# MiniXC/LightningFastSpeech2

Hardware: AMD Instinct MI355X
Metric: mel-frames/sec (whole node), 256-phoneme batch-32 (higher is better)
Workload: dtype bf16

## Files before the change

### include/fs2.h

```cpp
#ifndef FS2_H_
#define FS2_H_

#include <stddef.h>
#include <stdint.h>

#ifdef __cplusplus
extern "C" {
#endif

#define FS2_ABI_VERSION 4
#define FS2_MAX_LAYERS 32
#define FS2_MAX_VARIANCES 4
#define FS2_MAX_PRIORS 8
#define FS2_NAME_LEN 32

enum fs2_status {
    FS2_OK = 0,
    FS2_ERR_HIP = 1,
    FS2_ERR_SHAPE = 2,
    FS2_ERR_ARG = 3,
    FS2_ERR_WEIGHT = 4,
    FS2_ERR_STATE = 5,
    FS2_ERR_NOMEM = 6
};
// ... 105 lines not shown
int32_t fs2_op_vocoder_resblock_form(int32_t dtype, int32_t channels, int32_t taps, const int32_t* dilations, int32_t npairs);
int32_t fs2_op_vocoder_conv_tile(int32_t dtype, int32_t n, int32_t cin, int32_t taps, int32_t dil, int32_t shift, int32_t post,
                                 int32_t* cin_pad);
int fs2_op_gemm(int32_t dtype, int32_t out_dtype, const void* x, const void* w, const float* bias, void* c,
                int32_t M, int32_t N, int32_t Cin, int32_t taps, int32_t S, int32_t relu, void* hip_stream);
int fs2_op_gemm_relu_dropout(int32_t dtype, const void* x, const void* w, const float* bias, void* c, int32_t M, int32_t N, int32_t Cin,
                             int32_t taps, int32_t S, float p, uint64_t seed, uint64_t key, void* hip_stream);
int fs2_op_gemm_add(int32_t dtype, const void* x, const void* w, const float* bias, const void* addend, void* c, int32_t M, int32_t N,
                    int32_t Cin, int32_t taps, int32_t S, void* hip_stream);
int fs2_op_gemm_rowscale(const void* x, const void* w, const float* bias, const float* rowstats, const float* wg,
                         void* c, int32_t M, int32_t N, int32_t Cin, void* hip_stream);
int fs2_op_gemm_rowscale_dt(int32_t dtype, int32_t out_dtype, const void* x, const void* w, const float* bias, const float* rowstats,
                            const float* wg, void* c, int32_t M, int32_t N, int32_t Cin, void* hip_stream);
int fs2_op_gemm_stats(int32_t dtype, const void* x, const void* w, const float* bias, const void* res, void* c, float* stats, int32_t M,
                      int32_t N, int32_t Cin, int32_t relu, void* hip_stream);
int fs2_op_rowstats_finish(const float* parts, int32_t nparts, int32_t ncols, float eps, float* out, int32_t M, void* hip_stream);
int fs2_op_gemm_head(const void* x, const void* w, const float* bias, const float* head_gw, float* stats_out, float* head_out, int32_t M,
                     int32_t N, int32_t Cin, int32_t relu, void* hip_stream);
int fs2_op_head_finish(const float* parts, const float* dots, int32_t nparts, int32_t ncols, float eps, float sum_gw, float cst,
                       const uint8_t* mask, float* pred, int32_t M, void* hip_stream);
int fs2_op_gemm_splitk_choice(int32_t dtype, int32_t M, int32_t N, int32_t Cin, int32_t taps, int32_t S);
int32_t fs2_op_gemm_route(int32_t dtype, int32_t out_dtype, int32_t M, int32_t N, int32_t Cin, int32_t taps, int32_t S, int32_t ksplit,
                          uint32_t present, int32_t bias_aligned);
int fs2_op_gemm_splitk(int32_t dtype, int32_t out_dtype, const void* x, const void* w, void* c, float* part, int32_t M, int32_t N,
                       int32_t Cin, int32_t taps, int32_t S, int32_t ksplit, int32_t accumulate, void* hip_stream);
int fs2_op_gemm_gated(int32_t dtype, const void* x, const void* w, const float* bias, const void* gate, float scale, void* c,
                      int32_t M, int32_t N, int32_t Cin, int32_t taps, int32_t S, void* hip_stream);
int fs2_op_attention(int32_t dtype, const void* qkv, const uint8_t* key_pad_mask, void* out, void* vt_scratch,
                     uint64_t* bits_scratch, int32_t B, int32_t S, int32_t H, int32_t heads, void* hip_stream);
int fs2_op_attention_x3(const float* qkv, const uint8_t* key_pad_mask, float* out, void* split_scratch, uint64_t* bits_scratch,
                        int32_t B, int32_t S, int32_t H, int32_t heads, void* hip_stream);
int fs2_op_gemm_split_out(const void* x, const void* w, const float* bias, void* c_hi, void* c_lo, int32_t M, int32_t N, int32_t Cin,
                          int32_t split, void* hip_stream);
int fs2_op_gemm_ln(int32_t dtype, const void* x, const void* w, const float* bias, const void* res,
                   const float* ln_g, const float* ln_b, const float* dot_w, float dot_b, const uint8_t* mask,
                   float* pred, void* y, void* tmp, int32_t M, int32_t N, int32_t Cin, int32_t taps, int32_t S,
                   int32_t relu, void* hip_stream);
int fs2_op_gemm_ln_tape(int32_t dtype, const void* x, const void* w, const float* bias, const void* res, const float* ln_g,
                        const float* ln_b, void* y, void* z_out, int32_t M, int32_t N, int32_t Cin, int32_t taps, int32_t S,
                        int32_t relu, void* hip_stream);
int fs2_op_gemm_ln_tape_dropout(int32_t dtype, const void* x, const void* w, const float* bias, const void* res, const float* ln_g,
                                const float* ln_b, void* y, void* z_out, int32_t M, int32_t N, int32_t Cin, int32_t taps, int32_t S,
                                int32_t relu, float p, uint64_t seed, uint64_t key, void* hip_stream);
size_t fs2_op_attention_scratch_bytes(int32_t dtype, int32_t B, int32_t S, int32_t H, int32_t heads, size_t* bits_bytes);
int fs2_op_layernorm(int32_t dtype, const void* x, const void* res, const float* gamma, const float* beta, void* y,
                     const float* dot_w, float dot_b, const uint8_t* mask, float* pred, int32_t M, int32_t H,
// ... 243 lines not shown
```

### lightningfastspeech2_amd/csrc/capi_ops.hip

```cpp
#include <math.h>

#include "fs2_common.h"
#include "fs2_kernels.h"

using namespace fs2;

namespace fs2 {

template <typename S, typename D>
__global__ __launch_bounds__(256) void convert_kernel(const S* __restrict__ s, D* __restrict__ d, size_t n) {
    for (size_t i = (size_t)blockIdx.x * 256 + threadIdx.x; i < n; i += (size_t)gridDim.x * 256)
        d[i] = Num<D>::from_f32(Num<S>::to_f32(s[i]));
}

int launch_convert(const ConvertArgs& a, int sdt, int ddt, hipStream_t st) {
    if (a.n == 0) return FS2_OK;
    size_t blocks = (a.n + 255) / 256;
    if (blocks > 4096) blocks = 4096;
    const dim3 g((unsigned)blocks), b(256);
    if (sdt == FS2_F32 && ddt == FS2_F32) hipLaunchKernelGGL((convert_kernel<float, float>), g, b, 0, st, (const float*)a.src, (float*)a.dst, a.n);
    else if (sdt == FS2_F32 && ddt == FS2_BF16) hipLaunchKernelGGL((convert_kernel<float, bf16>), g, b, 0, st, (const float*)a.src, (bf16*)a.dst, a.n);
    else if (sdt == FS2_BF16 && ddt == FS2_F32) hipLaunchKernelGGL((convert_kernel<bf16, float>), g, b, 0, st, (const bf16*)a.src, (float*)a.dst, a.n);
    else if (sdt == FS2_BF16 && ddt == FS2_BF16) hipLaunchKernelGGL((convert_kernel<bf16, bf16>), g, b, 0, st, (const bf16*)a.src, (bf16*)a.dst, a.n);
    else if (sdt == FS2_F32 && ddt == FS2_F16) hipLaunchKernelGGL((convert_kernel<float, f16>), g, b, 0, st, (const float*)a.src, (f16*)a.dst, a.n);
// ... 4 lines not shown
}

}

namespace fs2 {
int apply_knob(Tuning& t, int variant) {
    int ok = 1;
    if (variant == 1500 || variant == 1501) t.attn_x3 = variant - 1500;
    else if (variant >= 1400 && variant <= 1402) t.gemm_wres = variant - 1400;
    else if (variant == 1340 || variant == 1341) t.enc_attn_out = variant - 1340;
    else if (variant == 1320 || variant == 1321) t.pred_fuse_embed = variant - 1320;
    else if (variant >= 1200 && variant <= 1204) t.attn_pipe = variant - 1200;
    else if (variant == 1100 || variant == 1101) t.colsum_fused = variant - 1100;
    else if (variant == 1000 || variant == 1001) t.bgemm_tn256 = variant - 1000;
    else if (variant >= 905 && variant <= 908) { if (variant >= 907) t.attn_bwd_nb_dq = 3 + ((variant - 905) & 1); else t.attn_bwd_nb = 3 + ((variant - 905) & 1); }
    else if (variant == 909) t.attn_bwd_nb = 1;
    else if (variant >= 900 && variant <= 903) { if (variant >= 902) t.attn_bwd_nb_dq = ((variant - 900) & 1) + 1; else t.attn_bwd_nb = ((variant - 900) & 1) + 1; }
    else if (variant == 904) t.attn_bwd_nb_dq = 0;
    else if (variant == 800 || variant == 801) t.bgemm_full = variant - 800;
    else if (variant == 700 || variant == 701) t.bgemm_xcd = variant - 700;
    else if (variant == 500 || variant == 501) t.split_f32 = variant - 500;
    else if (variant == 230 || variant == 231) t.head_sums = variant - 230;
    else if (variant == 220 || variant == 221) t.gemm_persist = variant - 220;
    else if (variant >= 200 && variant <= 202) t.slab_xcd_remap = variant - 200;
    else if (variant >= 0 && variant <= 7 && variant != 2) t.gemm_variant = variant;
    else ok = 0;
    if (!ok) return FS2_ERR_ARG;
    ++t.gen;
    return FS2_OK;
}
Tuning& op_tuning() {
    static thread_local Tuning t;
    return t;
}
}

static GemmArgs gemm_args(const void* x, const void* w, const float* bias, void* c, int M, int N, int Cin, int taps, int S, int relu) {
    GemmArgs a;
    a.X = x; a.W = w; a.bias = bias; a.C = c;
    a.M = M; a.N = N; a.K = taps * Cin; a.ldx = Cin; a.ldc = N;
    a.Cin = Cin; a.taps = taps; a.pad = (taps - 1) / 2; a.S = S; a.relu = relu;
    return a;
}

extern "C" {

// ... 122 lines not shown
    GemmArgs a = gemm_args(x, w, bias, c, M, N, Cin, 1, M, 0);
    a.rs_stats = rowstats; a.rs_wg = wg;
    return launch_gemm(a, dtype, out_dtype, (hipStream_t)stream);
}
int fs2_op_rowstats_finish(const float* parts, int32_t nparts, int32_t ncols, float eps, float* out, int32_t M, void* stream) {
    return launch_rowstats_finish(parts, nparts, ncols, eps, out, M, (hipStream_t)stream);
}
int fs2_op_gemm_head(const void* x, const void* w, const float* bias, const float* head_gw, float* stats_out, float* head_out, int32_t M,
                     int32_t N, int32_t Cin, int32_t relu, void* stream) {
    if (!x || !w || !bias || !head_gw || !stats_out || !head_out) return FS2_ERR_ARG;
    GemmArgs a = gemm_args(x, w, bias, nullptr, M, N, Cin, 1, M, relu);
    a.stats_out = stats_out; a.head_gw = head_gw; a.head_out = head_out; a.ln_eps = 1e-5f;
    return launch_gemm(a, FS2_BF16, FS2_BF16, (hipStream_t)stream);
}
int fs2_op_head_finish(const float* parts, const float* dots, int32_t nparts, int32_t ncols, float eps, float sum_gw, float cst,
                       const uint8_t* mask, float* pred, int32_t M, void* stream) {
    return launch_head_finish(parts, dots, nparts, ncols, eps, sum_gw, cst, mask, pred, M, (hipStream_t)stream);
}

int fs2_op_gemm_splitk_choice(int32_t dtype, int32_t M, int32_t N, int32_t Cin, int32_t taps, int32_t S) {
    return gemm_splitk_choice(M, N, Cin, taps, S, dtype);
}

int32_t fs2_op_gemm_route(int32_t dtype, int32_t out_dtype, int32_t M, int32_t N, int32_t Cin, int32_t taps, int32_t S, int32_t ksplit,
                          uint32_t present, int32_t bias_aligned) {
    static float dummy[8];
    void* p = (void*)(((uintptr_t)dummy + 15) & ~(uintptr_t)15);
    GemmArgs a = gemm_args(p, p, nullptr, p, M, N, Cin, taps, S, (present & GF_RELU) != 0);
    a.ksplit = ksplit;
    if (present & GF_BIAS) a.bias = (const float*)p + (bias_aligned ? 0 : 1);
    if (present & GF_RES) a.res = p;
    if (present & GF_LN) { a.ln_g = (const float*)p; a.ln_b = (const float*)p; }
    if (present & GF_DOT) a.dot_w = (const float*)p;
    if (present & GF_ZOUT) a.z_out = p;
    if (present & GF_LNTMP) a.ln_tmp = p;
    if (present & GF_STATS) a.stats_out = (float*)p;
    if (present & GF_EPIRES) a.epi_res = p;
    if (present & GF_GATE) a.gate = p;
    if (present & GF_DROP) a.drop_p = 0.1f;
    if (present & GF_RS) { a.rs_stats = (const float*)p; a.rs_wg = (const float*)p; }
    if (present & GF_HEAD) { a.head_out = (float*)p; a.head_gw = (const float*)p; }
    if (present & GF_ZR) a.zero_rows = (const uint8_t*)p;
    if (present & GF_CLO) a.C_lo = p;
    if (present & GF_SPLIT) a.split = 1;
    if (present & GF_WPRE) a.w_presplit = 1;
    const GemmRoute r = route_gemm(a, dtype, out_dtype);
    if (r.status != FS2_OK) return -r.status;
    return r.family | r.mi << 4 | (r.ln ? 1 : 0) << 8 | (r.split ? 1 : 0) << 9 | (r.defer ? 1 : 0) << 10 | (r.xpre ? 1 : 0) << 11 |
           (r.zr ? 1 : 0) << 12 | (r.presplit ? 1 : 0) << 13 | (r.two_launch ? 1 : 0) << 16;
}

int fs2_op_gemm_splitk(int32_t dtype, int32_t out_dtype, const void* x, const void* w, void* c, float* part, int32_t M, int32_t N,
                       int32_t Cin, int32_t taps, int32_t S, int32_t ksplit, int32_t accumulate, void* stream) {
    if (ksplit < 2 || !part) return FS2_ERR_ARG;
    GemmArgs a = gemm_args(x, w, nullptr, part, M, N, Cin, taps, S, 0);
    a.ksplit = ksplit;
    const int r = launch_gemm(a, dtype, FS2_F32, (hipStream_t)stream);
    if (r != FS2_OK) return r;
    return launch_split_k_reduce(part, c, (size_t)M * N, ksplit, accumulate, out_dtype, (hipStream_t)stream);
}

int fs2_op_gemm_gated(int32_t dtype, const void* x, const void* w, const float* bias, const void* gate, float scale, void* c, int32_t M,
                      int32_t N, int32_t Cin, int32_t taps, int32_t S, void* stream) {
    if (!gate) return FS2_ERR_ARG;
    GemmArgs a = gemm_args(x, w, bias, c, M, N, Cin, taps, S, 0);
    a.gate = gate; a.gate_scale = scale;
    return launch_gemm(a, dtype, dtype, (hipStream_t)stream);
}

int fs2_op_gemm_ln(int32_t dtype, const void* x, const void* w, const float* bias, const void* res,
                   const float* ln_g, const float* ln_b, const float* dot_w, float dot_b, const uint8_t* mask,
                   float* pred, void* y, void* tmp, int32_t M, int32_t N, int32_t Cin, int32_t taps, int32_t S,
// ... 399 lines not shown
```

### lightningfastspeech2_amd/csrc/fs2_kernels.h

```cpp
#pragma once
#include <hip/hip_runtime.h>
#include <stdint.h>

#include <type_traits>

#include "../../include/fs2.h"
#include "fs2_common.h"

namespace fs2 {

inline bool is_16bit(int dt) { return dt == FS2_BF16 || dt == FS2_F16; }
inline bool is_storage_dtype(int dt) { return dt == FS2_F32 || is_16bit(dt); }
inline bool is_f32_or_bf16(int dt) { return dt == FS2_F32 || dt == FS2_BF16; }
inline size_t elem_bytes(int dt) { return is_16bit(dt) ? 2 : 4; }

struct Tuning {
    int gemm_variant = 0;
    int gemm_wres = 1;
    int head_sums = 1;
    int gemm_persist = 1;
    int slab_xcd_remap = 1;
    int split_f32 = 0;
    int attn_pipe = 3;
    int attn_x3 = 1;
    int enc_attn_out = 1;
    int pred_fuse_embed = 1;
    int attn_bwd_nb = 1, attn_bwd_nb_dq = 0;
    int colsum_fused = 0;
    int bgemm_full = 1, bgemm_xcd = 1, bgemm_tn256 = 1;
    int voc_lds_limit = 0;
    int voc_fused_resblock = 1;
    unsigned long long gen = 0;
};
Tuning& op_tuning();
int apply_knob(Tuning& t, int variant);
inline const Tuning& tuning_of(const Tuning* t) { return t ? *t : op_tuning(); }

struct GemmArgs {
    const void* X;
    const void* W;
    const float* bias;
    void* C;
    void* C_lo = nullptr;
    int M, N, K;
// ... 22 lines not shown
    int w_presplit = 0;
    int split = 0;
    const uint8_t* zero_rows = nullptr;
    const void* gate = nullptr;
    float gate_scale = 1.f;
    float drop_p = 0.f;
    uint64_t drop_seed = 0, drop_key = 0;
    const float* rs_stats = nullptr;
    const float* rs_wg = nullptr;
    const float* head_gw = nullptr;
    float* head_out = nullptr;
    int ksplit = 0;
};
enum GemmFeature : unsigned {
    GF_BIAS = 1u << 0, GF_RES = 1u << 1, GF_LN = 1u << 2, GF_DOT = 1u << 3, GF_ZOUT = 1u << 4, GF_LNTMP = 1u << 5, GF_STATS = 1u << 6,
    GF_EPIRES = 1u << 7, GF_GATE = 1u << 8, GF_DROP = 1u << 9, GF_RS = 1u << 10 , GF_HEAD = 1u << 11 ,
    GF_ZR = 1u << 12, GF_CLO = 1u << 13, GF_SPLIT = 1u << 14, GF_WPRE = 1u << 15, GF_RELU = 1u << 16,
};
enum GemmFamily { GEMM_NONE = 0, GEMM_FLAT128 = 1, GEMM_SLAB = 2, GEMM_PERSIST = 3, GEMM_WRES = 4 };
struct GemmRoute {
    int status = FS2_OK;
    int family = GEMM_NONE;
    int mi = 0;
    int in_dtype = 0, out_dtype = 0;
    bool ln = false, split = false, defer = false, xpre = false;
    bool zr = false;
    bool two_launch = false;
    bool presplit = false;
};
inline bool layernorm_rows_ok(int H) { return H % 4 == 0 && H <= 1024; }
GemmRoute route_gemm(const GemmArgs& a, int in_dtype, int out_dtype);
int launch_route(const GemmRoute& r, const GemmArgs& a, hipStream_t stream);
inline int launch_gemm(const GemmArgs& a, int in_dtype, int out_dtype, hipStream_t stream) {
    return launch_route(route_gemm(a, in_dtype, out_dtype), a, stream);
}
int launch_presplit_pack(const float* w, void* out, size_t n_values, hipStream_t stream);
bool gemm_presplit_eligible(int N, int K);
int launch_split_k_reduce(const float* part, void* out, size_t n, int ksplit, int accumulate, int out_dtype, hipStream_t stream);
int gemm_splitk_choice(int M, int N, int Cin, int taps, int S, int in_dtype);
bool gemm_wres_supported(const GemmArgs& a, int in_dtype, int out_dtype, bool force);
int launch_gemm_wres(const GemmArgs& a, int dtype, hipStream_t stream);
bool gemm_persist_supported(const GemmArgs& a, int in_dtype, int out_dtype, int mi);
bool gemm_head_supported(const GemmArgs& a, int in_dtype, int out_dtype);
bool gemm_persist_pays(const GemmArgs& a, int mi);
int launch_gemm_persist(const GemmArgs& a, int dtype, int mi, hipStream_t stream);

// ... 529 lines not shown
```

### lightningfastspeech2_amd/csrc/gemm_mfma.hip

```cpp
#include <string.h>

#include "fs2_common.h"
#include "fs2_kernels.h"

namespace fs2 {

static constexpr int BM = 128, BN = 128, ROWB = 128;
static constexpr int TILE_BYTES = BM * ROWB;

__device__ inline int swz(int row, int slot) { return row * ROWB + ((slot ^ (row & 7)) << 4); }

template <typename T, typename OutT, bool ZR = false>
__global__ __launch_bounds__(256) void gemm_conv_kernel(GemmArgs p) {
    extern __shared__ __attribute__((aligned(16))) unsigned char smem[];
    unsigned char* sX = smem;
    unsigned char* sW = smem + 2 * TILE_BYTES;
    constexpr int E16 = Num<T>::kPer16B;
    constexpr int KE = ROWB / (int)sizeof(T);

    const int tid = threadIdx.x, lane = tid & 63, wave = tid >> 6;
    const int tiles_n = (p.N + BN - 1) / BN;
    const int bm = blockIdx.x / tiles_n, bn = blockIdx.x % tiles_n;
    const int m0 = bm * BM, n0 = bn * BN;

// ... 124 lines not shown
__device__ inline int wcol(int ni, int fgq) { return (ni >> 1) * 32 + fgq * 8 + (ni & 1) * 4; }
__device__ inline int wswz(int row) { return ((row >> 1) & 1) | (((row >> 3) & 3) << 1); }

template <int MI> struct SlabCfg {
    static constexpr int BM = MI * 32;
    static constexpr int SLAB_GROUPS = (BM + 30 + 7) / 8;
    static constexpr int SI = (SLAB_GROUPS + 7) / 8;
    static constexpr int SLAB_BYTES = SI * 8 * 1024;
};
static constexpr int S_BN = 256;
template <bool B> struct BoolC { static constexpr bool value = B; };

#ifdef FS2_SLAB_PROBE
__device__ unsigned long long g_slab_stamps[4][8];
#define SLAB_STAMP(i)                                                                                                   \
    do {                                                                                                                \
        if ((blockIdx.x == 0 || blockIdx.x == 128) && (threadIdx.x == 0 || threadIdx.x == 448))                          \
            g_slab_stamps[(blockIdx.x ? 2 : 0) + (threadIdx.x ? 1 : 0)][i] = __builtin_amdgcn_s_memtime();               \
    } while (0)
#else
#define SLAB_STAMP(i) do { } while (0)
#endif

template <typename T, typename OutT, int MI, bool LN, bool SPLIT = false, bool DEFER = false, bool XPRE = false>
__global__ __launch_bounds__(512) void gemm_conv_slab_kernel(GemmArgs p) {
    static_assert(!XPRE || SPLIT, "XPRE: the split arithmetic's conv form (activation slab split in place when it lands)");
    static_assert(!SPLIT || sizeof(T) == 4, "the split arithmetic takes fp32 operands");
    static_assert(!(DEFER && LN), "deferred LayerNorm is what a launch WITHOUT the fused epilogue leaves behind");
#if defined(__HIP_DEVICE_COMPILE__)
    using Cfg = SlabCfg<MI>;
    constexpr int BMs = Cfg::BM;
    constexpr int SI = Cfg::SI;
    constexpr int SLAB_B = Cfg::SLAB_BYTES;
    __shared__ __attribute__((aligned(16))) unsigned char slab0[SLAB_B];
    __shared__ __attribute__((aligned(16))) unsigned char slab1[SLAB_B];
    __shared__ __attribute__((aligned(16))) unsigned char wt0[S_BN * ROWB];
    __shared__ __attribute__((aligned(16))) unsigned char wt1[S_BN * ROWB];
    __shared__ __attribute__((aligned(16))) float sprm[(LN ? 4 : 1) * S_BN];
    constexpr int KE = ROWB / (int)sizeof(T);
    SLAB_STAMP(0);

    const int tid = threadIdx.x, lane = tid & 63;
    const int wave = __builtin_amdgcn_readfirstlane(tid >> 6);
    const int S = p.S, nutt = p.M / S;
    const int tiles_n = (p.N + S_BN - 1) / S_BN;
    const int tiles_m = (S + BMs - 1) / BMs;
    int bid = blockIdx.x;
    if (p.xcd_remap == 2) {
        const int ncg = tiles_n >> 1, xg = 8 / ncg, xcd = bid & 7, k = bid >> 3;
        bid = ((k >> 1) * xg + xcd / ncg) * tiles_n + (xcd % ncg) * 2 + (k & 1);
    } else if (p.xcd_remap) {
        const int nt = gridDim.x, per = nt >> 3, rem = nt & 7, xcd = bid & 7;
        bid = xcd * per + (xcd < rem ? xcd : rem) + (bid >> 3);
    }
    int ks = 0;
    if constexpr (!LN && !DEFER) {
        if (p.ksplit > 1) {
            const int per_split = gridDim.x / p.ksplit;
            ks = bid / per_split;
            bid -= ks * per_split;
        }
    }
    const int bn = bid % tiles_n;
    bid /= tiles_n;
    const int tm = bid % tiles_m, ub = bid / tiles_m;
    if (ub >= nutt) return;
    const int t0 = tm * BMs;
    int n0 = bn * S_BN;
    const int ntap = p.taps, ncc = p.Cin / KE / (p.ksplit > 1 ? p.ksplit : 1), cc0 = ks * ncc;
    const T* __restrict__ Xu = (const T*)p.X + (size_t)ub * S * p.ldx + cc0 * KE;
    constexpr unsigned OOB = 0xFFFFF000u;
    const unsigned xbytes = (unsigned)(((size_t)(S - 1) * p.ldx + p.Cin - cc0 * KE) * sizeof(T));
    const unsigned wbytes = (unsigned)((size_t)p.N * p.K * sizeof(T));
    const __amdgpu_buffer_rsrc_t xrs = __builtin_amdgcn_make_buffer_rsrc((void*)Xu, 0, xbytes, 0x00020000);
    const __amdgpu_buffer_rsrc_t wrs = __builtin_amdgcn_make_buffer_rsrc((void*)p.W, 0, wbytes, 0x00020000);
    constexpr int DW = 4, DSI = SI * 8 / DW, DWI = 32 / DW;
    const bool dma_wave = wave < DW;
    unsigned svoff[DSI];
#pragma unroll
    for (int i = 0; i < DSI; ++i) {
        const int P = (i * DW + (wave & (DW - 1))) * 64 + lane, row = P >> 3, ps = P & 7;
        const int t = t0 - p.pad + row;
        const bool ok = (t >= 0) & (t < S) & (row < BMs + ntap - 1);
        svoff[i] = ok ? (unsigned)t * (unsigned)(p.ldx * (int)sizeof(T)) + (unsigned)((ps ^ (row & 7)) << 4) : OOB;
    }
    unsigned wvoff[DWI];
    auto set_wvoff = [&]() {
#pragma unroll
        for (int i = 0; i < DWI; ++i) {
            const int P = (i * DW + (wave & (DW - 1))) * 64 + lane, row = P >> 3, ps = P & 7;
            const int n = n0 + row;
            wvoff[i] = n < p.N ? (unsigned)n * (unsigned)(p.K * (int)sizeof(T)) + (unsigned)((ps ^ wswz(row)) << 4) : OOB;
        }
    };
    set_wvoff();
    auto issue_slab = [&](unsigned char* dst, int cc) {
        if (!dma_wave) return;
#pragma unroll
        for (int i = 0; i < DSI; ++i)
            __builtin_amdgcn_raw_ptr_buffer_load_lds(xrs, (__attribute__((address_space(3))) void*)(dst + (i * DW + wave) * 1024),
                                                     16, svoff[i], cc * ROWB, 0, 0);
    };
    auto issue_w = [&](unsigned char* dst, int cc, int tap) {
        if (!dma_wave) return;
        const int koff = (tap * p.Cin + (cc0 + cc) * KE) * (int)sizeof(T);
#pragma unroll
        for (int i = 0; i < DWI; ++i)
            __builtin_amdgcn_raw_ptr_buffer_load_lds(wrs, (__attribute__((address_space(3))) void*)(dst + (i * DW + wave) * 1024),
                                                     16, wvoff[i], koff, 0, 0);
    };

    f32x4_t acc[4][MI];
    const int wm = wave >> 2, wn = wave & 3;
    const int fr = lane & 15, fg = lane >> 4;
    const int xrow0 = wm * (MI * 16) + fr;
    const bool res_in_acc = !p.relu && !(LN && p.drop_p > 0.f) && (LN ? p.res != nullptr : (DEFER && p.epi_res != nullptr));
    int woff[4][2];
#pragma unroll
    for (int i = 0; i < 4; ++i)
#pragma unroll
        for (int ks = 0; ks < 2; ++ks) {
            const int wrow = wn * 64 + wcol(i, fr >> 2) + (fr & 3);
            woff[i][ks] = wrow * ROWB + (((ks * 4 + fg) ^ wswz(wrow)) << 4);
        }

    auto compute = [&](const unsigned char* sl, const unsigned char* wt, int tap) {
        if constexpr (SPLIT) {
            uint4 wh[4], wl[4];
#pragma unroll
            for (int i = 0; i < 4; ++i) { wh[i] = *(const uint4*)(wt + woff[i][0]); wl[i] = *(const uint4*)(wt + woff[i][1]); }
            if constexpr (XPRE) {
                uint4 xh[2], xl[2];
// ... 51 lines not shown
            uint4 h, l;
            split_bf16x3(*(const uint4*)a0, *(const uint4*)a1, h, l);
            *(uint4*)a0 = h;
            *(uint4*)a1 = l;
        }
    };
#define FS2_SLAB_STEP(slab_cur, slab_nxt, w_cur, w_nxt, ccv, tapv)                          \
    {                                                                                       \
        dma_drain();          \
        __syncthreads();   \
        int ntp = (tapv) + 1, ncb = (ccv);                                                  \
        if (ntp == ntap) { ntp = 0; ++ncb; }                                                \
        if (ncb < ncc) issue_w(w_nxt, ncb, ntp);                                            \
        if ((tapv) == 0 && (ccv) + 1 < ncc) issue_slab(slab_nxt, (ccv) + 1);                \
        if constexpr (XPRE) {                                                               \
            if ((tapv) == 0) {                                                              \
                split_rows(slab_cur, BMs + ntap - 1);                                       \
                __syncthreads();                                                            \
            }                                                                               \
        }                                                                                   \
        compute(slab_cur, w_cur, (tapv));                                                   \
    }
    SLAB_STAMP(1);
    issue_slab(slab0, 0);
    issue_w(wt0, 0, 0);
    float prm[LN ? 4 : 1];
    if (tid < S_BN) {
        const int n = n0 + tid;
        const bool nv = n < p.N;
        prm[0] = (p.bias && nv) ? p.bias[n] : 0.f;
        if constexpr (LN) {
            prm[1] = nv ? p.ln_g[n] : 0.f;
            prm[2] = nv ? p.ln_b[n] : 0.f;
            prm[3] = (nv && p.dot_w) ? p.dot_w[n] : 0.f;
        }
    }
#pragma unroll
    for (int a = 0; a < 4; ++a)
#pragma unroll
        for (int b = 0; b < MI; ++b) acc[a][b] = (f32x4_t){0.f, 0.f, 0.f, 0.f};
    if ((LN || DEFER) && res_in_acc) {
        const T* R = (const T*)(LN ? p.res : p.epi_res) + (size_t)ub * S * p.ldc;
        const bool rnorm = DEFER && p.epi_res_stats != nullptr;
        const size_t rowbase0 = (size_t)ub * S;
        auto preload = [&](auto full_c) {
            constexpr bool FULL = decltype(full_c)::value;
            constexpr int GP = MI;
#pragma unroll
// ... 83 lines not shown
                            for (int r = 0; r < 8; ++r)
                                rv[r] = n + r < p.N ? __builtin_fmaf((rv[r] - rmean[gi]) * rrstd[gi], p.epi_res_g[n + r], p.epi_res_b[n + r]) : 0.f;
                        }
#pragma unroll
                        for (int r = 0; r < 8; ++r) acc[2 * j + (r >> 2)][g0 + gi][r & 3] = rv[r];
                    }
                }
            }
            if (MI > GP) __builtin_amdgcn_sched_barrier(0);
            }
        };
        if (n0 + S_BN <= p.N) preload(BoolC<true>{});
        else preload(BoolC<false>{});
    }
    if (tid < S_BN) {
        sprm[tid] = prm[0];
        if constexpr (LN) {
            sprm[S_BN + tid] = prm[1];
            sprm[2 * S_BN + tid] = prm[2];
            sprm[3 * S_BN + tid] = prm[3];
        }
    }
    SLAB_STAMP(6);
    for (int cc = 0; cc < ncc; cc += 2) {
        for (int tap = 0; tap < ntap; tap += 2) {
            FS2_SLAB_STEP(slab0, slab1, wt0, wt1, cc, tap)
            if (tap + 1 < ntap) FS2_SLAB_STEP(slab0, slab1, wt1, wt0, cc, tap + 1)
        }
        if (cc + 1 < ncc) {
            for (int tap = 0; tap < ntap; tap += 2) {
                FS2_SLAB_STEP(slab1, slab0, wt1, wt0, cc + 1, tap)
                if (tap + 1 < ntap) FS2_SLAB_STEP(slab1, slab0, wt0, wt1, cc + 1, tap + 1)
            }
        }
    }
    SLAB_STAMP(2);
#undef FS2_SLAB_STEP

    if constexpr (LN) {
        const size_t rowbase = (size_t)ub * S;
        const bool full = p.N == S_BN;
        {
            const float lo = p.relu ? 0.f : -__builtin_inff();
#pragma unroll
            for (int ni = 0; ni < 4; ++ni) {
                const int n = wn * 64 + wcol(ni, fg);
#pragma unroll
                for (int r = 0; r < 4; ++r) {
                    const float bvv = sprm[n + r];
#pragma unroll
                    for (int mi = 0; mi < MI; ++mi) acc[ni][mi][r] = fmaxf(acc[ni][mi][r] + bvv, lo);
                }
            }
            if (p.drop_p > 0.f) {
                const uint32_t thr = (uint32_t)(p.drop_p * 16777216.0f);
                const float dsc = 1.f / (1.f - p.drop_p);
#pragma unroll
// ... 382 lines not shown
    if (p.rs_stats) {
        if constexpr (sizeof(T) == 2 && sizeof(OutT) == 2 && !SPLIT) {
            if (fulln) store(BoolC<false>{}, BoolC<true>{}, BoolC<false>{}, BoolC<false>{}, BoolC<true>{});
            else store(BoolC<false>{}, BoolC<false>{}, BoolC<false>{}, BoolC<false>{}, BoolC<true>{});
        }
    } else if (p.gate) {
        if (fulln) store(BoolC<false>{}, BoolC<true>{}, BoolC<true>{}, BoolC<false>{}, BoolC<false>{});
        else store(BoolC<false>{}, BoolC<false>{}, BoolC<true>{}, BoolC<false>{}, BoolC<false>{});
    } else if (p.drop_p > 0.f) {
        if (fulln) store(BoolC<true>{}, BoolC<true>{}, BoolC<false>{}, BoolC<true>{}, BoolC<false>{});
        else store(BoolC<true>{}, BoolC<false>{}, BoolC<false>{}, BoolC<true>{}, BoolC<false>{});
    } else if (fulln) {
        if (p.relu) store(BoolC<true>{}, BoolC<true>{}, BoolC<false>{}, BoolC<false>{}, BoolC<false>{});
        else store(BoolC<false>{}, BoolC<true>{}, BoolC<false>{}, BoolC<false>{}, BoolC<false>{});
    } else {
        if (p.relu) store(BoolC<true>{}, BoolC<false>{}, BoolC<false>{}, BoolC<false>{}, BoolC<false>{});
        else store(BoolC<false>{}, BoolC<false>{}, BoolC<false>{}, BoolC<false>{}, BoolC<false>{});
    }
#else
    (void)p;
#endif
}

template <typename T, typename OutT, int MI, bool LN, bool SPLIT = false, bool DEFER = false, bool XPRE = false>
static int launch_slab_t(const GemmArgs& a0, hipStream_t stream) {
    GemmArgs a = a0;
    a.xcd_remap = tuning_of(a0.tune).slab_xcd_remap;
    const int BMs = SlabCfg<MI>::BM;
    if (a.xcd_remap == 2) {
        const int tn = (a.N + S_BN - 1) / S_BN, rows = (a.M / a.S) * ((a.S + BMs - 1) / BMs);
        const bool ok = (tn == 4 || tn == 8 || tn == 16) && a.ksplit <= 1 && rows % (16 / tn) == 0 &&
                        (size_t)a.N * a.K * sizeof(T) > (size_t)3 << 20;
        if (!ok) a.xcd_remap = 1;
    }
    if (a.taps == 1) a.S = a.M;
    const int tiles = (a.M / a.S) * ((a.S + BMs - 1) / BMs) * ((a.N + S_BN - 1) / S_BN) * (a.ksplit > 1 ? a.ksplit : 1);
    hipLaunchKernelGGL((gemm_conv_slab_kernel<T, OutT, MI, LN, SPLIT, DEFER, XPRE>), dim3(tiles), dim3(512), 0, stream, a);
    return hipGetLastError() == hipSuccess ? FS2_OK : FS2_ERR_HIP;
}

static int presplit_on_the_fly(GemmArgs& a, hipStream_t stream, void** tmp) {
    hipStreamCaptureStatus cs = hipStreamCaptureStatusNone;
    if (hipStreamIsCapturing(stream, &cs) != hipSuccess || cs != hipStreamCaptureStatusNone) return FS2_ERR_STATE;
    const size_t bytes = (size_t)a.N * a.K * 4;
    if (hipMallocAsync(tmp, bytes, stream) != hipSuccess) return FS2_ERR_NOMEM;
    const int r = launch_presplit_pack((const float*)a.W, *tmp, (size_t)a.N * a.K, stream);
    a.W = *tmp;
    a.w_presplit = 1;
    return r;
}

template <typename T, typename OutT, bool ZR = false>
static int launch_t(const GemmArgs& a, hipStream_t stream) {
    static bool attr_set = false;
    const size_t smem = 4 * TILE_BYTES;
    if (!attr_set) {
        hipError_t e = hipFuncSetAttribute((const void*)gemm_conv_kernel<T, OutT, ZR>,
                                           hipFuncAttributeMaxDynamicSharedMemorySize, (int)smem);
        if (e != hipSuccess) return FS2_ERR_HIP;
        attr_set = true;
// ... 62 lines not shown
    const Tuning& tn = tuning_of(a.tune);
    const int v = tn.gemm_variant, ke = 128 / (int)elem_bytes(in_dtype);
    const bool ln = a.ln_g != nullptr;
    const unsigned feats = (a.bias ? GF_BIAS : 0) | (a.relu ? GF_RELU : 0) | (ln ? GF_LN : 0) | (!ln && a.stats_out ? GF_STATS : 0) |
                           (!ln && a.epi_res ? GF_EPIRES : 0) | (!ln && a.drop_p > 0.f ? GF_DROP : 0) | (a.gate ? GF_GATE : 0) |
                           (a.rs_stats ? (a.N < 192 ? GF_RS_NARROW : GF_RS) : 0) | (a.zero_rows ? GF_ZR : 0) | (a.C_lo ? GF_CLO : 0) |
                           (a.w_presplit ? GF_WPRE : 0) | (a.ksplit > 1 ? GF_KSPLIT : 0);
    const unsigned have = (v == 0 ? ND_AUTO : 0) | (v != 1 ? ND_NOT_FLAT : 0) | (v == 0 || (v >= 3 && v <= 7) ? ND_SLAB_KNOB : 0) |
                          (a.N >= 192 ? ND_WIDE : 0) | (a.S > 0 && a.M % a.S == 0 && (a.taps & 1) ? ND_TILES : 0) |
                          (in_dtype == out_dtype ? ND_SAME_DT : 0) | (in_dtype == FS2_F32 ? ND_IN_F32 : 0) | (out_dtype == FS2_F32 ? ND_OUT_F32 : 0) |
                          (is_16bit(in_dtype) ? ND_IN_16 : 0) | (a.relu ? ND_RELU : 0) | (a.rs_wg ? ND_RS_WG : 0) | (a.taps == 1 ? ND_TAPS1 : 0) |
                          (a.split || tn.split_f32 ? ND_SPLIT_ON : 0) | (a.ksplit > 1 && (a.Cin / ke) % a.ksplit == 0 ? ND_KDIV : 0);
    return {feats, have};
}
static bool rules_hold(const Request& q, unsigned subject, int family) {
    for (const FeatureRule& r : kFeatureRules) {
        if (!(subject & r.feature)) continue;
        if ((q.feats & r.not_with) || (r.needs & ~q.have)) return false;
        if (family != GEMM_NONE && !(r.families & (1u << family))) return false;
    }
    return true;
}

static GemmRoute route_one(const GemmArgs& a, int in_dtype, int out_dtype) {
    GemmRoute r;
    if (a.M <= 0 || a.N <= 0) return r;
    const int ke = 128 / (int)elem_bytes(in_dtype), e16 = 16 / (int)elem_bytes(in_dtype);
    if (a.K % ke || a.Cin % ke || a.ldx % e16 || a.K != a.taps * a.Cin || a.ldc % 4) return GemmRoute{FS2_ERR_SHAPE};
    const Tuning& tn = tuning_of(a.tune);
    const Request q = classify(a, in_dtype, out_dtype);
    const bool ln = q.feats & GF_LN, defer = q.feats & (GF_STATS | GF_EPIRES), tiles_ok = q.have & ND_TILES;
    const int variant = tn.gemm_variant;
    const int ksp = a.ksplit > 1 ? a.ksplit : 1;
    const bool flat_only = q.feats & (GF_RS_NARROW | GF_ZR);
    const unsigned subject = flat_only ? q.feats & (GF_DROP | GF_RS_NARROW | GF_ZR) : q.feats;
    if (!rules_hold(q, subject, GEMM_NONE)) return GemmRoute{FS2_ERR_SHAPE};

    int family = GEMM_FLAT128, mi = 0;
    if (flat_only) {
    } else if (tiles_ok && (variant == 6 || variant == 7)) {
        family = GEMM_SLAB; mi = variant == 6 ? 1 : 2;
    } else if (tiles_ok && variant >= 3 && variant <= 5 && !(ln && variant == 5)) {
        family = GEMM_SLAB; mi = variant == 3 ? 4 : (variant == 4 || defer) ? 6 : 8;
    } else if (variant == 0 && tiles_ok && a.N >= 192) {
        const int S = a.taps == 1 ? a.M : a.S, nutt = a.M / S, tiles_n = (a.N + S_BN - 1) / S_BN;
        int best = 0;
// ... 5 lines not shown
            const long bm = h * 32, tm = (S + bm - 1) / bm;
            const long tiles = (long)nutt * tm * tiles_n * ksp;
            long cost = ((tiles + 255) / 256) * (bm + 40);
            if (a.K / ksp >= 4096) cost = cost > tiles ? cost : tiles;
            if (!best || cost < best_cost) { best = h; best_cost = cost; best_rows = (long)nutt * tm * bm; }
        }
        if (best_rows <= 2L * a.M || (q.feats & (GF_CLO | GF_WPRE | GF_RS))) {
            family = !ln && tn.gemm_persist && gemm_persist_supported(a, in_dtype, out_dtype, best) && gemm_persist_pays(a, best) ? GEMM_PERSIST : GEMM_SLAB;
            mi = best;
        }
    }
    if (ln && family != GEMM_SLAB) return r;
    if (!rules_hold(q, subject, family)) return GemmRoute{FS2_ERR_SHAPE};
    r.family = family; r.mi = mi;
    if (family == GEMM_FLAT128) {
        r.zr = q.feats & GF_ZR;
        if (!(dtype_pair(in_dtype, out_dtype) & flat_dtypes(r.zr))) return GemmRoute{FS2_ERR_SHAPE};
    } else if (family == GEMM_SLAB) {
        r.ln = ln; r.defer = defer;
        if (!(dtype_pair(in_dtype, out_dtype) & slab_dtypes(ln, defer))) return GemmRoute{FS2_ERR_SHAPE};
        r.split = in_dtype == FS2_F32 && out_dtype == FS2_F32 && (q.have & ND_SPLIT_ON);
        r.xpre = r.split && a.taps > 1;
        r.presplit = r.split && !a.w_presplit;
    }
    return r;
}

static GemmRoute route_request(const GemmArgs& a, int in_dtype, int out_dtype) {
    const auto no = [](int status) { return GemmRoute{status}; };
    const auto on = [](int family, int mi) { GemmRoute r; r.family = family; r.mi = mi; return r; };
    if (!is_storage_dtype(in_dtype) || !is_storage_dtype(out_dtype)) return no(FS2_ERR_ARG);
    if ((in_dtype == FS2_F16 || out_dtype == FS2_F16) && (a.drop_p > 0.f || a.gate || a.z_out || a.ksplit > 1 || a.head_out || a.C_lo)) return no(FS2_ERR_ARG);
    const Tuning& tn = tuning_of(a.tune);
    if (a.head_out) {
        if (a.ln_g || !gemm_head_supported(a, in_dtype, out_dtype)) return no(FS2_ERR_SHAPE);
        return on(GEMM_PERSIST, 6);
    }
    if (!a.ln_g) {
        if (a.drop_p > 0.f) {
            if (!rules_hold(classify(a, in_dtype, out_dtype), GF_DROP, GEMM_NONE)) return no(FS2_ERR_SHAPE);
        } else if (tn.gemm_wres && tn.gemm_variant == 0 && a.ksplit <= 1 && gemm_wres_supported(a, in_dtype, out_dtype, tn.gemm_wres == 2)) {
            return on(GEMM_WRES, 0);
        }
        return route_one(a, in_dtype, out_dtype);
    }
    if (a.z_out && a.N > S_BN) return no(FS2_ERR_SHAPE);
// ... 7 lines not shown
    GemmArgs g = a;
    g.ln_g = nullptr;
    g.C = a.ln_tmp;
    GemmRoute r = route_one(g, in_dtype, out_dtype);
    if (r.status != FS2_OK || r.family == GEMM_NONE) return r;
    if (!layernorm_rows_ok(a.N)) return no(FS2_ERR_SHAPE);
    r.two_launch = true;
    return r;
}
GemmRoute route_gemm(const GemmArgs& a, int in_dtype, int out_dtype) {
    GemmRoute r = route_request(a, in_dtype, out_dtype);
    r.in_dtype = in_dtype; r.out_dtype = out_dtype;
    return r;
}

template <int MI, bool LN, bool DEFER>
static int launch_slab_e(const GemmRoute& r, const GemmArgs& a, hipStream_t stream) {
    return with_dtypes<slab_dtypes(LN, DEFER)>(r.in_dtype, r.out_dtype, [&](auto t, auto o) {
        using T = typename decltype(t)::type;
        using OutT = typename decltype(o)::type;
        if constexpr (sizeof(T) == 4) {
            if (r.xpre) return launch_slab_t<T, OutT, MI, LN, true, DEFER, true>(a, stream);
            if (r.split) return launch_slab_t<T, OutT, MI, LN, true, DEFER>(a, stream);
        }
        return launch_slab_t<T, OutT, MI, LN, false, DEFER>(a, stream);
    });
}
template <int MI>
static int launch_slab_mi(const GemmRoute& r, const GemmArgs& a, hipStream_t stream) {
    if constexpr (MI <= 6) {
        if (r.ln) return launch_slab_e<MI, true, false>(r, a, stream);
        if (r.defer) return launch_slab_e<MI, false, true>(r, a, stream);
    }
    return launch_slab_e<MI, false, false>(r, a, stream);
}
template <bool ZR>
static int launch_flat(const GemmRoute& r, const GemmArgs& a, hipStream_t stream) {
    return with_dtypes<flat_dtypes(ZR)>(r.in_dtype, r.out_dtype, [&](auto t, auto o) {
        return launch_t<typename decltype(t)::type, typename decltype(o)::type, ZR>(a, stream);
    });
}

int launch_route(const GemmRoute& r, const GemmArgs& a_in, hipStream_t stream) {
    if (r.status != FS2_OK || r.family == GEMM_NONE) return r.status;
    GemmArgs a = a_in;
    if (r.two_launch) { a.ln_g = nullptr; a.C = a_in.ln_tmp; }
// ... 100 lines not shown
```

Baseline: 26.51 million.

## Add triple-buffered weight prefetch (lead-2) K loop to slab GEMM kernel

Adds a LEAD template mode to the slab conv/GEMM kernel. Weight tiles are triple-buffered so weight loads run two K steps ahead, with vmcnt-based waits limited to the DMA waves. Pointwise GEMMs (form 1) use a shrunk activation slab, and conv GEMMs with taps divisible by 3 (form 2) get their own stepping. The default knob turns it on only for a few specific shapes (mi=4 plain taps=9, mi=1 LN taps=3, mi=1 LN K=1024), at the cost of extra LDS and more complex synchronisation.

```diff
diff --git a/include/fs2.h b/include/fs2.h
--- a/include/fs2.h
+++ b/include/fs2.h
@@ -151,6 +151,8 @@
 int fs2_op_gemm_splitk_choice(int32_t dtype, int32_t M, int32_t N, int32_t Cin, int32_t taps, int32_t S);
 int32_t fs2_op_gemm_route(int32_t dtype, int32_t out_dtype, int32_t M, int32_t N, int32_t Cin, int32_t taps, int32_t S, int32_t ksplit,
                           uint32_t present, int32_t bias_aligned);
+int32_t fs2_op_gemm_route_lead(int32_t dtype, int32_t out_dtype, int32_t M, int32_t N, int32_t Cin, int32_t taps, int32_t S, int32_t ksplit,
+                               uint32_t present, int32_t bias_aligned);
 int fs2_op_gemm_splitk(int32_t dtype, int32_t out_dtype, const void* x, const void* w, void* c, float* part, int32_t M, int32_t N,
                        int32_t Cin, int32_t taps, int32_t S, int32_t ksplit, int32_t accumulate, void* hip_stream);
 int fs2_op_gemm_gated(int32_t dtype, const void* x, const void* w, const float* bias, const void* gate, float scale, void* c,
diff --git a/lightningfastspeech2_amd/csrc/capi_ops.hip b/lightningfastspeech2_amd/csrc/capi_ops.hip
--- a/lightningfastspeech2_amd/csrc/capi_ops.hip
+++ b/lightningfastspeech2_amd/csrc/capi_ops.hip
@@ -50,6 +50,7 @@
     else if (variant == 500 || variant == 501) t.split_f32 = variant - 500;
     else if (variant == 230 || variant == 231) t.head_sums = variant - 230;
     else if (variant == 220 || variant == 221) t.gemm_persist = variant - 220;
+    else if (variant >= 240 && variant <= 242) t.slab_lead = variant - 240;
     else if (variant >= 200 && variant <= 202) t.slab_xcd_remap = variant - 200;
     else if (variant >= 0 && variant <= 7 && variant != 2) t.gemm_variant = variant;
     else ok = 0;
@@ -218,8 +219,8 @@
     return gemm_splitk_choice(M, N, Cin, taps, S, dtype);
 }
 
-int32_t fs2_op_gemm_route(int32_t dtype, int32_t out_dtype, int32_t M, int32_t N, int32_t Cin, int32_t taps, int32_t S, int32_t ksplit,
-                          uint32_t present, int32_t bias_aligned) {
+static GemmRoute route_of_request(int32_t dtype, int32_t out_dtype, int32_t M, int32_t N, int32_t Cin, int32_t taps, int32_t S, int32_t ksplit,
+                                  uint32_t present, int32_t bias_aligned) {
     static float dummy[8];
     void* p = (void*)(((uintptr_t)dummy + 15) & ~(uintptr_t)15);
     GemmArgs a = gemm_args(p, p, nullptr, p, M, N, Cin, taps, S, (present & GF_RELU) != 0);
@@ -240,10 +241,21 @@
     if (present & GF_CLO) a.C_lo = p;
     if (present & GF_SPLIT) a.split = 1;
     if (present & GF_WPRE) a.w_presplit = 1;
-    const GemmRoute r = route_gemm(a, dtype, out_dtype);
+    return route_gemm(a, dtype, out_dtype);
+}
+int32_t fs2_op_gemm_route(int32_t dtype, int32_t out_dtype, int32_t M, int32_t N, int32_t Cin, int32_t taps, int32_t S, int32_t ksplit,
+                          uint32_t present, int32_t bias_aligned) {
+    const GemmRoute r = route_of_request(dtype, out_dtype, M, N, Cin, taps, S, ksplit, present, bias_aligned);
     if (r.status != FS2_OK) return -r.status;
     return r.family | r.mi << 4 | (r.ln ? 1 : 0) << 8 | (r.split ? 1 : 0) << 9 | (r.defer ? 1 : 0) << 10 | (r.xpre ? 1 : 0) << 11 |
            (r.zr ? 1 : 0) << 12 | (r.presplit ? 1 : 0) << 13 | (r.two_launch ? 1 : 0) << 16;
+}
+
+int32_t fs2_op_gemm_route_lead(int32_t dtype, int32_t out_dtype, int32_t M, int32_t N, int32_t Cin, int32_t taps, int32_t S, int32_t ksplit,
+                               uint32_t present, int32_t bias_aligned) {
+    const GemmRoute r = route_of_request(dtype, out_dtype, M, N, Cin, taps, S, ksplit, present, bias_aligned);
+    if (r.status != FS2_OK) return -r.status;
+    return r.family == GEMM_SLAB ? r.lead : 0;
 }
 
 int fs2_op_gemm_splitk(int32_t dtype, int32_t out_dtype, const void* x, const void* w, void* c, float* part, int32_t M, int32_t N,
diff --git a/lightningfastspeech2_amd/csrc/fs2_kernels.h b/lightningfastspeech2_amd/csrc/fs2_kernels.h
--- a/lightningfastspeech2_amd/csrc/fs2_kernels.h
+++ b/lightningfastspeech2_amd/csrc/fs2_kernels.h
@@ -20,6 +20,7 @@
     int head_sums = 1;
     int gemm_persist = 1;
     int slab_xcd_remap = 1;
+    int slab_lead = 1;
     int split_f32 = 0;
     int attn_pipe = 3;
     int attn_x3 = 1;
@@ -88,6 +89,7 @@
     int status = FS2_OK;
     int family = GEMM_NONE;
     int mi = 0;
+    int lead = 0;
     int in_dtype = 0, out_dtype = 0;
     bool ln = false, split = false, defer = false, xpre = false;
     bool zr = false;
diff --git a/lightningfastspeech2_amd/csrc/gemm_mfma.hip b/lightningfastspeech2_amd/csrc/gemm_mfma.hip
--- a/lightningfastspeech2_amd/csrc/gemm_mfma.hip
+++ b/lightningfastspeech2_amd/csrc/gemm_mfma.hip
@@ -170,20 +170,23 @@
 #define SLAB_STAMP(i) do { } while (0)
 #endif
 
-template <typename T, typename OutT, int MI, bool LN, bool SPLIT = false, bool DEFER = false, bool XPRE = false>
+template <typename T, typename OutT, int MI, bool LN, bool SPLIT = false, bool DEFER = false, bool XPRE = false, int LEAD = 0>
 __global__ __launch_bounds__(512) void gemm_conv_slab_kernel(GemmArgs p) {
     static_assert(!XPRE || SPLIT, "XPRE: the split arithmetic's conv form (activation slab split in place when it lands)");
+    static_assert(LEAD == 0 || (!SPLIT && sizeof(T) == 2), "the lead-2 K loop is the 16-bit kernels'");
+    static_assert(LEAD >= 0 && LEAD <= 2 && (LEAD != 2 || MI <= 4), "lead-2: pointwise (1) up to 192 rows, conv (2) up to 128 - what three weight stages leave of the LDS");
     static_assert(!SPLIT || sizeof(T) == 4, "the split arithmetic takes fp32 operands");
     static_assert(!(DEFER && LN), "deferred LayerNorm is what a launch WITHOUT the fused epilogue leaves behind");
 #if defined(__HIP_DEVICE_COMPILE__)
     using Cfg = SlabCfg<MI>;
     constexpr int BMs = Cfg::BM;
     constexpr int SI = Cfg::SI;
-    constexpr int SLAB_B = Cfg::SLAB_BYTES;
+    constexpr int SLAB_B = LEAD == 1 ? BMs * ROWB : Cfg::SLAB_BYTES;
     __shared__ __attribute__((aligned(16))) unsigned char slab0[SLAB_B];
     __shared__ __attribute__((aligned(16))) unsigned char slab1[SLAB_B];
     __shared__ __attribute__((aligned(16))) unsigned char wt0[S_BN * ROWB];
     __shared__ __attribute__((aligned(16))) unsigned char wt1[S_BN * ROWB];
+    __shared__ __attribute__((aligned(16))) unsigned char wt2[LEAD ? S_BN * ROWB : 16];
     __shared__ __attribute__((aligned(16))) float sprm[(LN ? 4 : 1) * S_BN];
     constexpr int KE = ROWB / (int)sizeof(T);
     SLAB_STAMP(0);
@@ -222,7 +225,7 @@
     const unsigned wbytes = (unsigned)((size_t)p.N * p.K * sizeof(T));
     const __amdgpu_buffer_rsrc_t xrs = __builtin_amdgcn_make_buffer_rsrc((void*)Xu, 0, xbytes, 0x00020000);
     const __amdgpu_buffer_rsrc_t wrs = __builtin_amdgcn_make_buffer_rsrc((void*)p.W, 0, wbytes, 0x00020000);
-    constexpr int DW = 4, DSI = SI * 8 / DW, DWI = 32 / DW;
+    constexpr int DW = 4, DSI = LEAD == 1 ? MI : SI * 8 / DW, DWI = 32 / DW;
     const bool dma_wave = wave < DW;
     unsigned svoff[DSI];
 #pragma unroll
@@ -256,6 +259,19 @@
         for (int i = 0; i < DWI; ++i)
             __builtin_amdgcn_raw_ptr_buffer_load_lds(wrs, (__attribute__((address_space(3))) void*)(dst + (i * DW + wave) * 1024),
                                                      16, wvoff[i], koff, 0, 0);
+    };
+    auto issue_slab_l = [&](unsigned char* dst, int cc, bool live) {
+#pragma unroll
+        for (int i = 0; i < DSI; ++i)
+            __builtin_amdgcn_raw_ptr_buffer_load_lds(xrs, (__attribute__((address_space(3))) void*)(dst + (i * DW + wave) * 1024),
+                                                     16, live ? svoff[i] : OOB, live ? cc * ROWB : 0, 0, 0);
+    };
+    auto issue_w_l = [&](unsigned char* dst, int cc, int tap, bool live) {
+        const int koff = live ? (tap * p.Cin + (cc0 + cc) * KE) * (int)sizeof(T) : 0;
+#pragma unroll
+        for (int i = 0; i < DWI; ++i)
+            __builtin_amdgcn_raw_ptr_buffer_load_lds(wrs, (__attribute__((address_space(3))) void*)(dst + (i * DW + wave) * 1024),
+                                                     16, live ? wvoff[i] : OOB, koff, 0, 0);
     };
 
     f32x4_t acc[4][MI];
@@ -353,8 +369,14 @@
         compute(slab_cur, w_cur, (tapv));                                                   \
     }
     SLAB_STAMP(1);
-    issue_slab(slab0, 0);
-    issue_w(wt0, 0, 0);
+    if constexpr (LEAD == 0) {
+        issue_slab(slab0, 0);
+        issue_w(wt0, 0, 0);
+    } else if (dma_wave) {
+        issue_slab_l(slab0, 0, true);
+        issue_w_l(wt0, 0, 0, true);
+        issue_w_l(wt1, ntap == 1 ? 1 : 0, ntap == 1 ? 0 : 1, ncc * ntap > 1);
+    }
     float prm[LN ? 4 : 1];
     if (tid < S_BN) {
         const int n = n0 + tid;
@@ -484,6 +506,7 @@
         }
     }
     SLAB_STAMP(6);
+    if constexpr (LEAD == 0) {
     for (int cc = 0; cc < ncc; cc += 2) {
         for (int tap = 0; tap < ntap; tap += 2) {
             FS2_SLAB_STEP(slab0, slab1, wt0, wt1, cc, tap)
@@ -495,6 +518,79 @@
                 if (tap + 1 < ntap) FS2_SLAB_STEP(slab1, slab0, wt0, wt1, cc + 1, tap + 1)
             }
         }
+    }
+    } else {
+        const int nsteps = ncc * ntap;
+        auto kloop = [&](auto dmaw_c) {
+            constexpr bool DMAW = decltype(dmaw_c)::value;
+#define FS2_LEAD_WAIT(cnt)                                                                                              \
+              \
+              \
+            __builtin_amdgcn_s_waitcnt(DMAW ? (0x0070 | (cnt)) : 0xC07F);                                               \
+            __builtin_amdgcn_s_barrier();
+            if constexpr (LEAD == 1) {
+#define FS2_LEAD_STEP(slab_cur, slab_nxt, w_cur, w_nn, sv)                                                              \
+                {                                                                                                       \
+                    FS2_LEAD_WAIT(DWI)                                                                                  \
+                    if constexpr (DMAW) {                                                                               \
+                        issue_slab_l(slab_nxt, (sv) + 1, (sv) + 1 < nsteps);                                            \
+                        issue_w_l(w_nn, (sv) + 2, 0, (sv) + 2 < nsteps);                                                \
+                    }                                                                                                   \
+                    compute(slab_cur, w_cur, 0);                                                                        \
+                }
+                FS2_LEAD_STEP(slab0, slab1, wt0, wt2, 0)
+                for (int s = 1; s < nsteps; s += 6) {
+                    FS2_LEAD_STEP(slab1, slab0, wt1, wt0, s)
+                    if (s + 1 >= nsteps) break;
+                    FS2_LEAD_STEP(slab0, slab1, wt2, wt1, s + 1)
+                    if (s + 2 >= nsteps) break;
+                    FS2_LEAD_STEP(slab1, slab0, wt0, wt2, s + 2)
+                    if (s + 3 >= nsteps) break;
+                    FS2_LEAD_STEP(slab0, slab1, wt1, wt0, s + 3)
+                    if (s + 4 >= nsteps) break;
+                    FS2_LEAD_STEP(slab1, slab0, wt2, wt1, s + 4)
+                    if (s + 5 >= nsteps) break;
+                    FS2_LEAD_STEP(slab0, slab1, wt0, wt2, s + 5)
+                }
+#undef FS2_LEAD_STEP
+            } else {
+#define FS2_LEAD_STEP(slab_cur, slab_nxt, w_cur, w_nn, ccv, tapv, cnt, slab_req)                                        \
+                {                                                                                                       \
+                    FS2_LEAD_WAIT(cnt)                                                                                  \
+                    if constexpr (DMAW) {                                                                               \
+                        int t2 = (tapv) + 2, c2 = (ccv);                                                                \
+                        if (t2 >= ntap) { t2 -= ntap; ++c2; }                                                           \
+                        issue_w_l(w_nn, c2, t2, c2 < ncc);                                                              \
+                        if constexpr (slab_req) issue_slab_l(slab_nxt, (ccv) + 1, (ccv) + 1 < ncc);                     \
+                    }                                                                                                   \
+                    compute(slab_cur, w_cur, (tapv));                                                                   \
+                }
+#define FS2_LEAD_BLOCK(slab_cur, slab_nxt, ccv)                                                                         \
+                {                                                                                                       \
+                    FS2_LEAD_STEP(slab_cur, slab_nxt, wt0, wt2, ccv, 0, DWI, true)                                      \
+                    FS2_LEAD_STEP(slab_cur, slab_nxt, wt1, wt0, ccv, 1, DWI + DSI, false)                               \
+                    FS2_LEAD_STEP(slab_cur, slab_nxt, wt2, wt1, ccv, 2, DWI + DSI, false)                               \
+                    for (int tap = 3; tap < ntap; tap += 3) {                                                           \
+                        FS2_LEAD_STEP(slab_cur, slab_nxt, wt0, wt2, ccv, tap, DWI, false)                               \
+                        FS2_LEAD_STEP(slab_cur, slab_nxt, wt1, wt0, ccv, tap + 1, DWI, false)                           \
+                        FS2_LEAD_STEP(slab_cur, slab_nxt, wt2, wt1, ccv, tap + 2, DWI, false)                           \
+                    }                                                                                                   \
+                }
+                static_assert(DWI + DSI <= 15, "vmcnt's low four bits");
+                for (int cc = 0;; cc += 2) {
+                    FS2_LEAD_BLOCK(slab0, slab1, cc)
+                    if (cc + 1 >= ncc) break;
+                    FS2_LEAD_BLOCK(slab1, slab0, cc + 1)
+                    if (cc + 2 >= ncc) break;
+                }
+#undef FS2_LEAD_BLOCK
+#undef FS2_LEAD_STEP
+            }
+#undef FS2_LEAD_WAIT
+        };
+        if (dma_wave) kloop(BoolC<true>{});
+        else kloop(BoolC<false>{});
+        dma_drain();
     }
     SLAB_STAMP(2);
 #undef FS2_SLAB_STEP
@@ -923,7 +1019,7 @@
 #endif
 }
 
-template <typename T, typename OutT, int MI, bool LN, bool SPLIT = false, bool DEFER = false, bool XPRE = false>
+template <typename T, typename OutT, int MI, bool LN, bool SPLIT = false, bool DEFER = false, bool XPRE = false, int LEAD = 0>
 static int launch_slab_t(const GemmArgs& a0, hipStream_t stream) {
     GemmArgs a = a0;
     a.xcd_remap = tuning_of(a0.tune).slab_xcd_remap;
@@ -936,7 +1032,7 @@
     }
     if (a.taps == 1) a.S = a.M;
     const int tiles = (a.M / a.S) * ((a.S + BMs - 1) / BMs) * ((a.N + S_BN - 1) / S_BN) * (a.ksplit > 1 ? a.ksplit : 1);
-    hipLaunchKernelGGL((gemm_conv_slab_kernel<T, OutT, MI, LN, SPLIT, DEFER, XPRE>), dim3(tiles), dim3(512), 0, stream, a);
+    hipLaunchKernelGGL((gemm_conv_slab_kernel<T, OutT, MI, LN, SPLIT, DEFER, XPRE, LEAD>), dim3(tiles), dim3(512), 0, stream, a);
     return hipGetLastError() == hipSuccess ? FS2_OK : FS2_ERR_HIP;
 }
 
@@ -1045,6 +1141,15 @@
     return true;
 }
 
+static int slab_lead_form(int knob, const GemmArgs& a, int in_dtype, int out_dtype, int mi, bool ln, bool defer) {
+    if (!knob || !is_16bit(in_dtype) || out_dtype != in_dtype || a.ksplit > 1) return 0;
+    const bool plain = !ln && !defer;
+    const int form = a.taps == 1 ? (mi <= 4 || (mi == 6 && plain) ? 1 : 0) : (a.taps % 3 == 0 && mi <= 4 ? 2 : 0);
+    if (knob >= 2 || !form) return form;
+    if (form == 2) return (mi == 4 && plain && a.taps == 9) || (mi == 1 && ln && a.taps == 3) ? 2 : 0;
+    return mi == 1 && ln && a.K == 1024 ? 1 : 0;
+}
+
 static GemmRoute route_one(const GemmArgs& a, int in_dtype, int out_dtype) {
     GemmRoute r;
     if (a.M <= 0 || a.N <= 0) return r;
@@ -1096,6 +1201,7 @@
         r.split = in_dtype == FS2_F32 && out_dtype == FS2_F32 && (q.have & ND_SPLIT_ON);
         r.xpre = r.split && a.taps > 1;
         r.presplit = r.split && !a.w_presplit;
+        r.lead = slab_lead_form(tn.slab_lead, a, in_dtype, out_dtype, mi, ln, defer);
     }
     return r;
 }
@@ -1149,6 +1255,13 @@
         if constexpr (sizeof(T) == 4) {
             if (r.xpre) return launch_slab_t<T, OutT, MI, LN, true, DEFER, true>(a, stream);
             if (r.split) return launch_slab_t<T, OutT, MI, LN, true, DEFER>(a, stream);
+        } else if constexpr (sizeof(OutT) == 2 && MI <= 6) {
+            if constexpr (MI <= 4 || (!LN && !DEFER)) {
+                if (r.lead == 1) return launch_slab_t<T, OutT, MI, LN, false, DEFER, false, 1>(a, stream);
+            }
+            if constexpr (MI <= 4) {
+                if (r.lead == 2) return launch_slab_t<T, OutT, MI, LN, false, DEFER, false, 2>(a, stream);
+            }
         }
         return launch_slab_t<T, OutT, MI, LN, false, DEFER>(a, stream);
     });
```

New measurement: 27.03 million (median of 6 runs). 2.0% higher.
